# wenxuanliu/multimodal-vae

Measured on AMD Instinct MI355X. Metric: ELBO-steps/sec (whole node), MultiMNIST b=256 per GPU, higher is better.
Workload: dtype bf16; 1 GPU; multimnist_50x50_conv_mmvae_gru_text_3pass_elbo_step; batch_per_gpu=256, global_batch=256, n_latents=100, parallelism=dp1, hip_graph=False, optimizer=adam, mfma=bf16 in / fp32 acc; fp32 master weights, BN stats, PoE/KL/BCE/NLL, Adam

## Files before the change

### include/mmvae_hip.h

```cpp
#ifndef MMVAE_HIP_H
#define MMVAE_HIP_H
#include <stddef.h>
#include <stdint.h>

#ifdef __cplusplus
extern "C" {
#endif

#define MMVAE_OK 0
#define MMVAE_EINVAL (-1)
#define MMVAE_EHIP (-2)
#define MMVAE_ENOSPC (-3)
#define MMVAE_ESTATE (-4)
#define MMVAE_ETIMEOUT (-5)

int mmvae_init(int device);
const char* mmvae_last_error(void);
const char* mmvae_version(void);
int mmvae_set_stream_policy(int flat);

typedef struct mmvae_comm mmvae_comm_t;
int mmvae_comm_unique_id(void* out128);
int mmvae_comm_init(mmvae_comm_t** out, int rank, int world, const void* unique_id128);
int mmvae_allreduce_grads(mmvae_comm_t*, float* flat, size_t n, void* stream);
// ... 64 lines not shown
int mmvae_mm_image_decoder_fwd(mmvae_mm_t*, void* ws, size_t ws_bytes, const float* z, int training, float* recon,
                               void* stream);
int mmvae_mm_image_decoder_bwd(mmvae_mm_t*, void* ws, size_t ws_bytes, const float* d_recon, const float* recon,
                               float* dz, void* stream);
int mmvae_mm_text_encoder_fwd(mmvae_mm_t*, void* ws, size_t ws_bytes, const long long* text, float* out_mu_logvar,
                              void* stream);
int mmvae_mm_text_encoder_bwd(mmvae_mm_t*, void* ws, size_t ws_bytes, const long long* text, const float* d_out,
                              void* stream);
int mmvae_mm_text_decoder_fwd(mmvae_mm_t*, void* ws, size_t ws_bytes, const float* z, int training, const uint8_t* keep,
                              const long long* force_tokens, float* words, long long* tokens, void* stream);
int mmvae_mm_text_decoder_bwd(mmvae_mm_t*, void* ws, size_t ws_bytes, const float* z, const uint8_t* keep,
                              const long long* force_tokens, const float* words, const long long* tokens,
                              const float* d_words, float* dz, void* stream);
size_t mmvae_mm_iw_workspace_bytes(const mmvae_mm_t*);
int mmvae_mm_iw_score(mmvae_mm_t*, void* ws, size_t ws_bytes, const float* z, const float* image, int B, int K, float* loglik_x,
                      float* words, void* stream);
int mmvae_mm_bench_layer(mmvae_mm_t*, void* ws, size_t ws_bytes, const char* layer, int iters, void* stream);
double mmvae_mm_layer_flops(const mmvae_mm_t*, const char* layer);
double mmvae_mm_layer_algo_flops(const mmvae_mm_t*, const char* layer);
double mmvae_mm_layer_algo_bytes(const mmvae_mm_t*, const char* layer);
double mmvae_debug_flops(int reset);
int mmvae_debug_set(const char* key, int value);
long long mmvae_mm_debug_offset(mmvae_mm_t*, const char* name);

typedef struct MnistPlan mmvae_mnist_t;
mmvae_mnist_t* mmvae_mnist_create(int n_latents, int batch);
mmvae_mnist_t* mmvae_mnist_create_p(int n_latents, int batch, int precision);
int mmvae_mnist_precision(const mmvae_mnist_t*);
void mmvae_mnist_destroy(mmvae_mnist_t*);
long long mmvae_mnist_param_count(const mmvae_mnist_t*);
int mmvae_mnist_num_params(const mmvae_mnist_t*);
int mmvae_mnist_param_info(const mmvae_mnist_t*, int i, char* name128, int* ndim, int* shape4, long long* offset);
long long mmvae_mnist_bn_floats(const mmvae_mnist_t*);
int mmvae_mnist_num_bn(const mmvae_mnist_t*);
int mmvae_mnist_bn_info(const mmvae_mnist_t*, int i, char* prefix128, int* channels, long long* offset);
long long mmvae_mnist_packed_elems(const mmvae_mnist_t*);
long long mmvae_mnist_packed_vec_elems(const mmvae_mnist_t*);
long long mmvae_mnist_gpk_elems(const mmvae_mnist_t*);
long long mmvae_mnist_gpk_vec_elems(const mmvae_mnist_t*);
size_t mmvae_mnist_desc_bytes(const mmvae_mnist_t*, int which);
int mmvae_mnist_desc_copy(const mmvae_mnist_t*, int which, void* host_out);
size_t mmvae_mnist_workspace_bytes(const mmvae_mnist_t*);
size_t mmvae_mnist_module_workspace_bytes(const mmvae_mnist_t*);
int mmvae_mnist_bind(mmvae_mnist_t*, float* params, float* grads, float* bn_stats, long long* num_batches_tracked,
                     void* packed_bf16, float* packed_vec, float* gpk, float* gpk_vec, void* desc_dev, void* gdesc_dev);
int mmvae_mnist_pack_weights(mmvae_mnist_t*, void* stream);
// ... 446 lines not shown
```

### multimodal-vae_amd/csrc/capi.cpp

```cpp
#include "../../include/mmvae_hip.h"
#include "multimnist.h"
#include "mmtext.h"
#include "mnist.h"
#include "mnist_plan.h"
#include "mnist_strip.h"
#include "celeba.h"
#include "coco.h"
#include "plan_base.h"
#include "iw.h"
#include "nn_words.h"
#include "mmd.h"
#include "tsne.h"
#include "pixelcnn.h"
#include "causal_conv.h"
#include "head_nll.h"
#include "conv4s2.h"
#include "multimnist_gen.h"
#include "imgprep.h"
#include <cstring>
#include <exception>

const char* mmvae_error_string();

template <class F>
// ... 153 lines not shown
}
size_t mmvae_mm_iw_workspace_bytes(const mmvae_mm_t* p) { return mm_b(p)->ws_bytes_module; }
int mmvae_mm_iw_score(mmvae_mm_t* p, void* ws, size_t wsb, const float* z, const float* image, int B, int K, float* loglik_x,
                      float* words, void* stream) {
    return guarded([&] { return mm_iw_score(p, ws, wsb, z, image, B, K, loglik_x, words, S(stream)); });
}
int mmvae_mm_image_step(mmvae_mm_t* p, const mmvae_image_step_io* io, int training, int do_backward, void* stream) {
    return guarded([&]() -> int {
        MMVAE_REQUIRE(p && io, "mmvae_mm_image_step: null argument");
        return mm_image_step(p, *io, training, do_backward, S(stream));
    });
}
size_t mmvae_mm_image_step_workspace_bytes(const mmvae_mm_t* p) { return p ? mm_image_step_workspace_bytes(p) : 0; }
int mmvae_mm_iw_score_image(mmvae_mm_t* p, void* ws, size_t wsb, const float* z, const float* image, int B, int K, float* loglik_x, void* st) {
    return guarded([&] { return mm_iw_score_image(p, ws, wsb, z, image, B, K, loglik_x, S(st)); });
}
int mmvae_mm_bench_layer(mmvae_mm_t* p, void* ws, size_t wsb, const char* layer, int iters, void* stream) {
    return guarded([&] { return mm_bench_layer(p, ws, wsb, layer, iters, S(stream)); });
}
double mmvae_mm_layer_flops(const mmvae_mm_t* p, const char* layer) { return mm_layer_flops(p, layer); }
double mmvae_mm_layer_algo_flops(const mmvae_mm_t* p, const char* layer) { return mm_layer_algo_flops(p, layer); }
double mmvae_mm_layer_algo_bytes(const mmvae_mm_t* p, const char* layer) { return mm_layer_algo_bytes(p, layer); }
long long mmvae_mm_debug_offset(mmvae_mm_t* p, const char* name) { return mm_debug_offset(p, name); }

mmvae_mmtext_t* mmvae_mmtext_create(int n_latents, int n_hiddens, int batch) {
    try { return mmtext_create(n_latents, n_hiddens, batch); } catch (...) { mmvae_set_error("mmtext_create failed"); return nullptr; }
}
void mmvae_mmtext_destroy(mmvae_mmtext_t* p) { mmtext_destroy(p); }
int mmvae_mmtext_hidden(const mmvae_mmtext_t* p) { return mmtext_hidden(p); }
MMVAE_PLAN_API(mmtext, mmvae_mmtext_t, mmtext_b)
int mmvae_mmtext_step(mmvae_mmtext_t* p, const mmvae_mm_text_step_io* io, int training, int do_backward, void* stream) {
    return guarded([&]() -> int {
        MMVAE_REQUIRE(p && io, "mmvae_mmtext_step: null argument");
        return mmtext_step(p, *io, training, do_backward, S(stream));
    });
}
int mmvae_mmtext_encoder_fwd(mmvae_mmtext_t* p, void* ws, size_t wsb, const long long* text, float* out, void* stream) {
    return guarded([&] { return mmtext_encoder_fwd(p, ws, wsb, text, out, S(stream)); });
}
int mmvae_mmtext_encoder_bwd(mmvae_mmtext_t* p, void* ws, size_t wsb, const long long* text, const float* d_out, void* stream) {
    return guarded([&] { return mmtext_encoder_bwd(p, ws, wsb, text, d_out, S(stream)); });
}
int mmvae_mmtext_decoder_fwd(mmvae_mmtext_t* p, void* ws, size_t wsb, const float* z, int training, const uint8_t* keep,
                             const long long* force_tokens, float* words, long long* tokens, void* stream) {
    return guarded([&] { return mmtext_decoder_fwd(p, ws, wsb, z, training, keep, force_tokens, words, tokens, S(stream)); });
}
// ... 886 lines not shown
```

### multimodal-vae_amd/csrc/elementwise.h

```cpp
#pragma once
#include "common.h"

struct PackDesc {
    long long dst_off;
    long long src_off;
    int Npad, Kpad, N, K;
    int NL;
    int s_nhi, s_nlo;
    int TW, C;
    int s_ty, s_tx, s_c;
    int o_ty, o_tx, step_t;
    int is_f32;
    long long bias_off;
    int b_nhi, b_nlo;
    int first_block;
    int part;
    int frag;
};

int launch_pack(const PackDesc* table_dev, const PackDesc* table_host, int ndesc, const float* params,
                bf16* packed_bf, float* packed_f32, hipStream_t s);
int launch_pack_range(const PackDesc* table_dev, const PackDesc* table_host, int ndesc, int d0, int d1, const float* params,
                      bf16* packed_bf, float* packed_f32, hipStream_t s);
int launch_unpack_grads(const PackDesc* table_dev, const PackDesc* table_host, int ndesc, const float* gpk_mat,
                        const float* gpk_vec, float* grads_flat, hipStream_t s, int part = -1);

int launch_im2col_small(const float* src, int Nimg, int Cin, int H, int W, int KH, int KW, int stride, int pad,
                        int OH, int OW, bf16* dst, int ld, hipStream_t s);

struct BnFinalizeArgs {
    const float2* stats;
    int G, C;
    float count;
    const float* gamma; const float* beta;
    float* running_mean; float* running_var; long long* num_batches_tracked;
    int updates_per_group;
    unsigned skip_update_mask;
    float2* affine;
    float2* meanrstd;
    float eps, momentum;
    int training;
// ... 126 lines not shown
    const int* gmap; const float* gpk; const float* gpk_vec; float* g_out;
    int nr; long long roff[4], rlen[4]; int no_advance;
};
int launch_adam(const AdamArgs& a, hipStream_t s);
int launch_gather_rows(const void* src, const long long* idx, long long rows, long long row_bytes, void* dst, hipStream_t s);
int launch_gather_rows_u8_f32(const unsigned char* src, const long long* idx, long long rows, long long row_elems, float denom, float* dst, hipStream_t s);
struct StepLossArgs { const float* sums; float* out; float w_bce[3], w_nll[3], w_kl[3]; };
int launch_step_losses(const StepLossArgs& a, hipStream_t s);
int launch_unpack_map(const PackDesc* table_dev, const PackDesc* table_host, int nd, long long nparams, long long gmat_elems, int* map, hipStream_t s);
int launch_fill_zero(void* p, size_t bytes, hipStream_t s);
int launch_bce_fwd(const float* p, const float* t, long long n, float* out, hipStream_t s);
int launch_bce_bwd(const float* p, const float* t, long long n, float coef, const float* gscale, float* dp, hipStream_t s);
int launch_nll_fwd(const float* lp, const long long* tg, int rows, int classes, float* out, hipStream_t s);
int launch_nll_bwd(const long long* tg, int rows, int classes, float coef, const float* gscale, float* dlp, hipStream_t s);

struct StepBeginArgs {
    void* zero_ptr[4]; size_t zero_bytes[4];
    float* eps; long long n_eps;
    uint8_t* mask[3]; long long n_mask[3];
    float p;
    unsigned long long seed; const long long* step;
    const PackDesc* pack_table; int pack_nd; const float* pack_params; bf16* packed_bf; float* packed_f32; int pack_blocks;
    unsigned pack_parts;
};
int launch_step_begin(const StepBeginArgs& a, hipStream_t s);
int step_begin_with_pack(StepBeginArgs& a, const PackDesc* table_dev, const PackDesc* table_host, int nd, const float* params,
                         bf16* packed_bf, float* packed_f32);

int launch_embed_gather_stats(const float* table, int C, const long long* idx, int rows, int idx_rows, int rows_per_group,
                              bf16* x, int ld, float2* colstats, hipStream_t s);
int launch_embed_scatter_add(const bf16* d, int ld, int C, const long long* idx, int rows, float* g_table, hipStream_t s);
struct LogSoftmaxNllArgs {
    const float* logits; int rows, classes;
    float* words;
    const long long* target; int target_rows; int rows_per_group;
    float* nll_sum;
    bf16* dlogits; int ld_d;
    float* dlogits_f32;
    float coef[4];
};
int launch_logsoftmax_nll(const LogSoftmaxNllArgs& a, hipStream_t s);
int launch_cast_bf16(const float* x, long long n, bf16* out, hipStream_t s);
int launch_colsum_f32(const float* x, int rows, int cols, float* out, hipStream_t s);
int launch_colsum_bf16(const bf16* x, int ld, int rows, int cols, float* out, hipStream_t s);
int launch_u8_to_f32(const uint8_t* src, long long n, float denom, float* dst, hipStream_t s);
int launch_mse_fwd(const float* a, const float* b, long long n, float* out_sum, hipStream_t s);
int launch_mse_bwd(const float* a, const float* b, long long n, float coef, const float* gscale, float* d_a, hipStream_t s);
```

### multimodal-vae_amd/csrc/elementwise.hip

```cpp
#include "elementwise.h"
#include "bn_dev.h"
#include <math.h>

namespace {

constexpr int TPB = 256;

__device__ __forceinline__ float exp_unfused(float x) {
    const float c = 0x1.715476p+0f, cc = 0x1.4ae0bep-26f;
    float ph = x * c;
    asm volatile("" : "+v"(ph));
    float pl = fmaf(x, c, -ph);
    pl = fmaf(x, cc, pl);
    const float e = rintf(ph);
    float r = ldexpf(__builtin_amdgcn_exp2f((ph - e) + pl), (int)e);
    r = x < -0x1.9d1dap+6f ? 0.f : r;
    r = x > 0x1.62e43p+6f ? INFINITY : r;
    return r;
}
inline int nblocks(long long n, int per = TPB, int cap = 4096) {
    long long b = (n + per - 1) / per;
    if (b < 1) b = 1;
    if (b > cap) b = cap;
    return (int)b;
}

__device__ __forceinline__ int find_desc(const PackDesc* t, int nd, int block) {
    const int lane = threadIdx.x & 63;
    int found = 0;
    for (int base = 0; base < nd; base += 64) {
        const int i = base + lane;
        const bool le = i < nd && t[i].first_block <= block;
        const unsigned long long m = __ballot(le);
        found += __popcll(m);
        if (m != ~0ull) break;
    }
    return __builtin_amdgcn_readfirstlane(found > 0 ? found - 1 : 0);
}
__device__ __forceinline__ int fast_divmod_ew(int r, int d, float inv, int& rem) {
    int q = (int)((float)r * inv);
    rem = r - q * d;
    if (rem < 0) { --q; rem += d; }
    else if (rem >= d) { ++q; rem -= d; }
    return q;
}
__device__ __forceinline__ long long pack_src(const PackDesc& d, int n, int k) {
    int nhi = n / d.NL, nlo = n - nhi * d.NL;
    int tap = k / d.C, c = k - tap * d.C;
    int ty = tap / d.TW, tx = tap - ty * d.TW;
    return d.src_off + (long long)nhi * d.s_nhi + (long long)nlo * d.s_nlo +
           (long long)(d.o_ty + ty * d.step_t) * d.s_ty + (long long)(d.o_tx + tx * d.step_t) * d.s_tx + (long long)c * d.s_c;
}

__device__ __forceinline__ void pack_block(const PackDesc* __restrict__ table, int nd, const float* __restrict__ params,
                                           bf16* __restrict__ packed_bf, float* __restrict__ packed_f32, int block, unsigned parts = 0u) {
    const int di = find_desc(table, nd, block);
    const PackDesc d = table[di];
    if (parts != 0u && !((parts >> (d.part & 31)) & 1u)) return;
    const int v = (int)(block - d.first_block) * TPB + threadIdx.x;
    const int vpr = d.Kpad / 8;
    if (v >= d.Npad * vpr) return;
    int kv;
    const int n = fast_divmod_ew(v, vpr, 1.0f / (float)vpr, kv);
    const int k0 = kv * 8;
    float val[8];
#pragma unroll
    for (int j = 0; j < 8; ++j) val[j] = 0.f;
    if (n < d.N) {
        int nlo;
        const int nhi = fast_divmod_ew(n, d.NL, 1.0f / (float)d.NL, nlo);
        const long long rowbase = d.src_off + (long long)nhi * d.s_nhi + (long long)nlo * d.s_nlo;
        if (d.C % 8 == 0 && k0 + 8 <= d.K) {
            int c, tx;
            const int tap = fast_divmod_ew(k0, d.C, 1.0f / (float)d.C, c);
            const int ty = fast_divmod_ew(tap, d.TW, 1.0f / (float)d.TW, tx);
            const long long b = rowbase + (long long)(d.o_ty + ty * d.step_t) * d.s_ty + (long long)(d.o_tx + tx * d.step_t) * d.s_tx + (long long)c * d.s_c;
#pragma unroll
            for (int j = 0; j < 8; ++j) val[j] = params[b + (long long)j * d.s_c];
        } else {
#pragma unroll
            for (int j = 0; j < 8; ++j) {
                const int k = k0 + j;
                if (k < d.K) val[j] = params[pack_src(d, n, k)];
                else if (k == d.K && d.bias_off >= 0) val[j] = params[d.bias_off + (long long)nhi * d.b_nhi + (long long)nlo * d.b_nlo];
            }
        }
    }
    const long long e = d.frag ? ((long long)((n >> 4) * (d.Kpad >> 5) + (kv >> 2)) * 64 + (kv & 3) * 16 + (n & 15)) * 8 : (long long)n * d.Kpad + k0;
    if (d.is_f32) {
#pragma unroll
        for (int j = 0; j < 8; ++j) packed_f32[d.dst_off + e + j] = val[j];
    } else {
        bf16x8 o;
#pragma unroll
        for (int j = 0; j < 8; ++j) o[j] = (bf16)val[j];
        *reinterpret_cast<bf16x8*>(packed_bf + d.dst_off + e) = o;
    }
}

__global__ __launch_bounds__(TPB) void pack_kernel(const PackDesc* __restrict__ table, int nd, const float* __restrict__ params,
                                                   bf16* __restrict__ packed_bf, float* __restrict__ packed_f32, int block0) {
    pack_block(table, nd, params, packed_bf, packed_f32, block0 + blockIdx.x);
}

template <bool MAP>
__global__ __launch_bounds__(TPB) void unpack_kernel(const PackDesc* __restrict__ table, int nd, const float* __restrict__ gmat,
                                                     const float* __restrict__ gvec, float* __restrict__ grads, int* __restrict__ map,
                                                     int part) {
    const int di = find_desc(table, nd, blockIdx.x);
    const PackDesc d = table[di];
    if (part >= 0 && d.part != part) return;
    const int v = (int)(blockIdx.x - d.first_block) * TPB + threadIdx.x;
    const int vpr = d.Kpad / 8;
    if (v >= d.N * vpr) return;
    int kv, nlo;
    const int n = fast_divmod_ew(v, vpr, 1.0f / (float)vpr, kv);
    const int k0 = kv * 8;
    if (k0 > d.K) return;
    const int nhi = fast_divmod_ew(n, d.NL, 1.0f / (float)d.NL, nlo);
    const long long sidx = d.dst_off + (long long)n * d.Kpad + k0;
    float val[8] = {0.f, 0.f, 0.f, 0.f, 0.f, 0.f, 0.f, 0.f};
    if (!MAP) {
        const float* src = (d.is_f32 ? gvec : gmat) + sidx;
        const f32x4 lo = *reinterpret_cast<const f32x4*>(src), hi = *reinterpret_cast<const f32x4*>(src + 4);
#pragma unroll
// ... 307 lines not shown
    for (long long q = (long long)blockIdx.x * TPB + threadIdx.x; q * 4 < n; q += (long long)gridDim.x * TPB) {
        uint32_t r[4];
        Philox::gen(seed ^ (st * 0x9E3779B97F4A7C15ull), (uint64_t)q, stream_id, r);
        float u0 = u01(r[0]), u1 = u01(r[1]), u2 = u01(r[2]), u3 = u01(r[3]);
        float m0 = sqrtf(-2.0f * logf(u0)), m1 = sqrtf(-2.0f * logf(u2));
        float v[4] = {m0 * cosf(6.28318530718f * u1), m0 * sinf(6.28318530718f * u1),
                      m1 * cosf(6.28318530718f * u3), m1 * sinf(6.28318530718f * u3)};
        for (int j = 0; j < 4; ++j)
            if (q * 4 + j < n) out[q * 4 + j] = v[j];
    }
}
__global__ __launch_bounds__(TPB) void keep_mask_kernel(uint8_t* out, long long n, float p, unsigned long long seed, const long long* step, unsigned stream_id) {
    const unsigned long long st = step ? (unsigned long long)*step : 0ull;
    for (long long q = (long long)blockIdx.x * TPB + threadIdx.x; q * 4 < n; q += (long long)gridDim.x * TPB) {
        uint32_t r[4];
        Philox::gen(seed ^ (st * 0x9E3779B97F4A7C15ull), (uint64_t)q, stream_id, r);
        for (int j = 0; j < 4; ++j)
            if (q * 4 + j < n) out[q * 4 + j] = u01(r[j]) >= p ? 1 : 0;
    }
}

__global__ __launch_bounds__(TPB) void step_begin_kernel(const StepBeginArgs a) {
    if ((int)blockIdx.x < a.pack_blocks) {
        pack_block(a.pack_table, a.pack_nd, a.pack_params, a.packed_bf, a.packed_f32, blockIdx.x, a.pack_parts);
        return;
    }
    const long long gtid = (long long)(blockIdx.x - a.pack_blocks) * TPB + threadIdx.x, gstride = (long long)(gridDim.x - a.pack_blocks) * TPB;
#pragma unroll
    for (int r = 0; r < 4; ++r) {
        if (!a.zero_ptr[r]) continue;
        u32x4* p = reinterpret_cast<u32x4*>(a.zero_ptr[r]);
        const long long n16 = (long long)(a.zero_bytes[r] / 16);
        for (long long i = gtid; i < n16; i += gstride) p[i] = u32x4{0u, 0u, 0u, 0u};
    }
    const unsigned long long st = a.step ? (unsigned long long)*a.step : 0ull;
    const unsigned long long key = a.seed ^ (st * 0x9E3779B97F4A7C15ull);
    if (a.eps) {
        for (long long q = gtid; q * 4 < a.n_eps; q += gstride) {
            uint32_t r[4];
            Philox::gen(key, (uint64_t)q, 1, r);
            float u0 = u01(r[0]), u1 = u01(r[1]), u2 = u01(r[2]), u3 = u01(r[3]);
            float m0 = sqrtf(-2.0f * logf(u0)), m1 = sqrtf(-2.0f * logf(u2));
            float v[4] = {m0 * cosf(6.28318530718f * u1), m0 * sinf(6.28318530718f * u1),
                          m1 * cosf(6.28318530718f * u3), m1 * sinf(6.28318530718f * u3)};
            for (int j = 0; j < 4; ++j)
                if (q * 4 + j < a.n_eps) a.eps[q * 4 + j] = v[j];
        }
// ... 489 lines not shown
}

}

int launch_mse_fwd(const float* a, const float* b, long long n, float* out, hipStream_t s) {
    hipLaunchKernelGGL(mse_fwd_kernel, dim3(nblocks(n, TPB * 4, 256)), dim3(TPB), 0, s, a, b, n, out);
    return mmvae_check_launch("mse_fwd");
}
int launch_mse_bwd(const float* a, const float* b, long long n, float coef, const float* gs, float* da, hipStream_t s) {
    hipLaunchKernelGGL(mse_bwd_kernel, dim3((unsigned)((n + TPB - 1) / TPB)), dim3(TPB), 0, s, a, b, n, coef, gs, da);
    return mmvae_check_launch("mse_bwd");
}
int launch_u8_to_f32(const uint8_t* src, long long n, float denom, float* dst, hipStream_t s) {
    MMVAE_REQUIRE(src && dst && n >= 0, "u8_to_f32: null argument");
    if (n == 0) return MMVAE_OK;
    hipLaunchKernelGGL(u8_to_f32_kernel, dim3((unsigned)((n + 16 * TPB - 1) / (16 * TPB))), dim3(TPB), 0, s, src, n, denom, dst);
    return mmvae_check_launch("u8_to_f32");
}
int launch_pack(const PackDesc* table_dev, const PackDesc* table_host, int nd, const float* params, bf16* packed_bf,
                float* packed_f32, hipStream_t s) {
    MMVAE_REQUIRE(nd > 0, "pack: empty table");
    for (int i = 0; i < nd; ++i)
        MMVAE_REQUIRE((long long)table_host[i].Npad * (table_host[i].Kpad / 8) < (1 << 23), "pack: matrix %d too large for 32-bit index math", i);
    hipLaunchKernelGGL(pack_kernel, dim3(table_blocks(table_host, nd)), dim3(TPB), 0, s, table_dev, nd, params, packed_bf, packed_f32, 0);
    return mmvae_check_launch("pack");
}
int launch_pack_range(const PackDesc* table_dev, const PackDesc* table_host, int nd, int d0, int d1, const float* params, bf16* packed_bf,
                      float* packed_f32, hipStream_t s) {
    MMVAE_REQUIRE(0 <= d0 && d0 <= d1 && d1 <= nd, "pack: descriptor range [%d, %d) of %d", d0, d1, nd);
    if (d0 == d1) return MMVAE_OK;
    const int b0 = (int)table_host[d0].first_block, b1 = d1 < nd ? (int)table_host[d1].first_block : table_blocks(table_host, nd);
    hipLaunchKernelGGL(pack_kernel, dim3(b1 - b0), dim3(TPB), 0, s, table_dev, nd, params, packed_bf, packed_f32, b0);
    return mmvae_check_launch("pack");
}
int launch_unpack_grads(const PackDesc* table_dev, const PackDesc* table_host, int nd, const float* gmat, const float* gvec,
                        float* grads, hipStream_t s, int part) {
    MMVAE_REQUIRE(nd > 0, "unpack: empty table");
    for (int i = 0; i < nd; ++i)
        MMVAE_REQUIRE((long long)table_host[i].Npad * (table_host[i].Kpad / 8) < (1 << 23), "unpack: matrix %d too large for 32-bit index math", i);
    hipLaunchKernelGGL(unpack_kernel<false>, dim3(table_blocks(table_host, nd)), dim3(TPB), 0, s, table_dev, nd, gmat, gvec, grads, (int*)nullptr, part);
    return mmvae_check_launch("unpack_grads");
}
int launch_unpack_map(const PackDesc* table_dev, const PackDesc* table_host, int nd, long long nparams, long long gmat_elems, int* map, hipStream_t s) {
    MMVAE_REQUIRE(nd > 0 && map, "unpack_map: empty table");
    MMVAE_REQUIRE(gmat_elems < (1ll << 31) - 2, "unpack_map: packed gradient buffer too large for 32-bit indices");
    if (hipMemsetAsync(map, 0xFF, (size_t)nparams * sizeof(int), s) != hipSuccess) { mmvae_set_error("hipMemsetAsync failed"); return MMVAE_EHIP; }
    hipLaunchKernelGGL(unpack_kernel<true>, dim3(table_blocks(table_host, nd)), dim3(TPB), 0, s, table_dev, nd, (const float*)nullptr,
                       (const float*)nullptr, (float*)nullptr, map, -1);
    return mmvae_check_launch("unpack_map");
}
int launch_im2col_small(const float* src, int Nimg, int Cin, int H, int W, int KH, int KW, int stride, int pad, int OH, int OW,
                        bf16* dst, int ld, hipStream_t s) {
    MMVAE_REQUIRE(ld % 8 == 0 && ld >= KH * KW * Cin && ld / 8 <= TPB, "im2col: ld=%d", ld);
    MMVAE_REQUIRE((long long)Nimg * OH * OW < (1 << 23) && (long long)Cin * H * W < (1ll << 31), "im2col: too many rows");
    const int rpb = TPB / (ld / 8);
// ... 215 lines not shown
    return MMVAE_OK;
}

int launch_bce_fwd(const float* p, const float* t, long long n, float* out, hipStream_t s) {
    hipLaunchKernelGGL(bce_fwd_kernel, dim3(nblocks(n, TPB * 4, 1024)), dim3(TPB), 0, s, p, t, n, out);
    return mmvae_check_launch("bce_fwd");
}
int launch_bce_bwd(const float* p, const float* t, long long n, float coef, const float* gs, float* dp, hipStream_t s) {
    hipLaunchKernelGGL(bce_bwd_kernel, dim3((unsigned)((n + TPB - 1) / TPB)), dim3(TPB), 0, s, p, t, n, coef, gs, dp);
    return mmvae_check_launch("bce_bwd");
}
int launch_nll_fwd(const float* lp, const long long* tg, int rows, int classes, float* out, hipStream_t s) {
    hipLaunchKernelGGL(nll_fwd_kernel, dim3(nblocks(rows, TPB, 64)), dim3(TPB), 0, s, lp, tg, rows, classes, out);
    return mmvae_check_launch("nll_fwd");
}
int launch_nll_bwd(const long long* tg, int rows, int classes, float coef, const float* gs, float* dlp, hipStream_t s) {
    hipLaunchKernelGGL(nll_bwd_kernel, dim3(ceil_div(rows * classes, TPB)), dim3(TPB), 0, s, tg, rows, classes, coef, gs, dlp);
    return mmvae_check_launch("nll_bwd");
}

int launch_step_begin(const StepBeginArgs& a, hipStream_t s) {
    for (int r = 0; r < 4; ++r)
        MMVAE_REQUIRE(a.zero_ptr[r] == nullptr || (a.zero_bytes[r] % 16 == 0 && ((uintptr_t)a.zero_ptr[r] & 15) == 0), "step_begin: zero range %d is not 16-byte aligned", r);
    MMVAE_LAUNCH(step_begin_kernel, dim3(mmvae_knob("begin_blocks", 2048) + (a.pack_blocks > 0 ? a.pack_blocks : 0)), dim3(TPB), 0, s, a);
    return mmvae_check_launch("step_begin");
}
int step_begin_with_pack(StepBeginArgs& a, const PackDesc* table_dev, const PackDesc* table_host, int nd, const float* params,
                         bf16* packed_bf, float* packed_f32) {
    MMVAE_REQUIRE(nd > 0, "pack: empty table");
    for (int i = 0; i < nd; ++i)
        MMVAE_REQUIRE((long long)table_host[i].Npad * (table_host[i].Kpad / 8) < (1 << 23), "pack: matrix %d too large for 32-bit index math", i);
    a.pack_table = table_dev; a.pack_nd = nd; a.pack_params = params; a.packed_bf = packed_bf; a.packed_f32 = packed_f32;
    a.pack_blocks = table_blocks(table_host, nd);
    return MMVAE_OK;
}

int launch_embed_gather_stats(const float* table, int C, const long long* idx, int rows, int idx_rows, int rows_per_group,
                              bf16* x, int ld, float2* colstats, hipStream_t s) {
    MMVAE_REQUIRE(C >= 1 && ld >= C && ld % 8 == 0, "embed_gather: C=%d ld=%d", C, ld);
    MMVAE_REQUIRE(rows >= 1 && idx_rows >= 1 && rows_per_group >= 1 && table && idx && x, "embed_gather: rows=%d idx_rows=%d rows_per_group=%d or a null argument",
                  rows, idx_rows, rows_per_group);
    hipLaunchKernelGGL(embed_gather_stats_kernel, dim3(ceil_div(rows, 64)), dim3(TPB), 0, s, table, C, idx, rows, idx_rows, rows_per_group, x, ld, colstats);
    return mmvae_check_launch("embed_gather_stats");
}
int launch_embed_scatter_add(const bf16* d, int ld, int C, const long long* idx, int rows, float* g_table, hipStream_t s) {
    MMVAE_REQUIRE(rows >= 1 && C >= 1 && ld >= C && (long long)rows * C <= 0x3FFFFFFF && d && idx && g_table, "embed_scatter: rows=%d C=%d ld=%d or a null argument",
                  rows, C, ld);
    hipLaunchKernelGGL(embed_scatter_add_kernel, dim3(ceil_div(rows * C, TPB)), dim3(TPB), 0, s, d, ld, C, idx, rows, g_table);
    return mmvae_check_launch("embed_scatter_add");
}
int launch_logsoftmax_nll(const LogSoftmaxNllArgs& a, hipStream_t s) {
    MMVAE_REQUIRE(a.rows >= 1 && a.classes >= 1 && a.rows_per_group >= 1 && a.logits && a.words, "logsoftmax_nll: rows=%d classes=%d rows_per_group=%d or a null argument",
                  a.rows, a.classes, a.rows_per_group);
    MMVAE_REQUIRE(ceil_div(a.rows, a.rows_per_group) <= 4, "logsoftmax_nll: %d rows are more than 4 groups of %d", a.rows, a.rows_per_group);
    MMVAE_REQUIRE(!a.target || a.target_rows >= 1, "logsoftmax_nll: target_rows=%d", a.target_rows);
    MMVAE_REQUIRE(!a.dlogits || a.ld_d >= a.classes, "logsoftmax_nll: ld_d=%d < classes=%d", a.ld_d, a.classes);
// ... 23 lines not shown
```

### multimodal-vae_amd/csrc/multimnist.h

```cpp
#pragma once
#include "layers.h"
#include "text.h"
#include "../../include/mmvae_hip.h"

struct PlanBase;

struct MMPlan;
int mm_early_ranges(const MMPlan* P, long long* ranges, int cap);
MMPlan* mm_create(int D, int B);
void mm_destroy(MMPlan*);
PlanBase* mm_base(MMPlan*);
int mm_step_fwd_bwd(MMPlan*, const mmvae_mm_step_io&, int training, int do_backward, hipStream_t);
int mm_image_encoder_fwd(MMPlan*, void* ws, size_t wsb, const float* image, const uint8_t* m1, const uint8_t* m2,
                         int training, float* out, hipStream_t);
int mm_image_encoder_bwd(MMPlan*, void* ws, size_t wsb, const float* d_out, const uint8_t* m1, const uint8_t* m2, hipStream_t);
int mm_image_decoder_fwd(MMPlan*, void* ws, size_t wsb, const float* z, int training, float* recon, hipStream_t);
int mm_image_decoder_bwd(MMPlan*, void* ws, size_t wsb, const float* d_recon, const float* recon, float* dz, hipStream_t);
int mm_text_encoder_fwd(MMPlan*, void* ws, size_t wsb, const long long* text, float* out, hipStream_t);
int mm_text_encoder_bwd(MMPlan*, void* ws, size_t wsb, const long long* text, const float* d_out, hipStream_t);
int mm_text_decoder_fwd(MMPlan*, void* ws, size_t wsb, const float* z, int training, const uint8_t* keep,
                        const long long* force_tokens, float* words, long long* tokens, hipStream_t);
int mm_text_decoder_bwd(MMPlan*, void* ws, size_t wsb, const float* z, const uint8_t* keep, const long long* force_tokens,
                        const float* words, const long long* tokens, const float* d_words, float* dz, hipStream_t);
int mm_iw_score(MMPlan*, void* ws, size_t wsb, const float* z, const float* image, int B, int K, float* loglik_x, float* words,
                hipStream_t);
int mm_image_step(MMPlan*, const mmvae_image_step_io&, int training, int do_backward, hipStream_t);
size_t mm_image_step_workspace_bytes(const MMPlan*);
int mm_iw_score_image(MMPlan*, void* ws, size_t wsb, const float* z, const float* image, int B, int K, float* loglik_x, hipStream_t);
int mm_wait_early_grads(MMPlan*, hipStream_t s);
int mm_bench_layer(MMPlan*, void* ws, size_t wsb, const char* layer, int iters, hipStream_t);
double mm_layer_flops(const MMPlan*, const char* layer);
double mm_layer_algo_flops(const MMPlan*, const char* layer);
double mm_layer_algo_bytes(const MMPlan*, const char* layer);
long long mm_debug_offset(MMPlan*, const char* name);
```

### multimodal-vae_amd/csrc/multimnist.hip

```cpp
#include "multimnist.h"
#include <memory>
#include "mlp_tail.h"
#include "plan_base.h"
#include "thin.h"
#include "text_plan.h"
#include <cstring>

namespace {
constexpr int IMG = 50, NPIX = 2500;
}

struct MMPlan : PlanBase {
    int ldz, kx, kz;
    int lde;
    ConvL conv[4], convT[4];
    LinL fc[3], up;
    BnL bn[6];
    int H = TXT_H;
    const char *te_name = "text_encoder", *td_name = "text_decoder";
    TextGruIdx te_f, te_r, td0, td1;
    const float* step_image = nullptr;
    hipEvent_t ev_dz = nullptr;
    hipEvent_t ev_txtgrads = nullptr;
    int te_h2p, te_h2pT, g_te_h2p, td_z2h, td_z2hT, g_td_z2h, td_h2o, td_h2oT, g_td_h2o;
// ... 705 lines not shown
    const uint8_t *m1 = io.enc_mask1, *m2 = io.enc_mask2, *gk = io.gru_keep;
    const bool serial0 = mmvae_serial();
    const bool staged = mmvae_knob("mm_stage_begin", 1) != 0 && !serial0;
    StepBeginArgs sb{}, sb2{};
    sb.zero_ptr[0] = w.zero_begin; sb.zero_bytes[0] = w.zero_bytes;
    StepBeginArgs& sz = staged ? sb2 : sb;
    if (do_backward) {
        sz.zero_ptr[1] = P.buf.gpk; sz.zero_bytes[1] = (size_t)P.gk.mat_elems * sizeof(float);
        sz.zero_ptr[2] = P.buf.grads; sz.zero_bytes[2] = (size_t)(P.nparams / 4) * 16;
        const int skipz = mmvae_knob("dbg_begin_skip_zero", 0);
        if (skipz & 1) sz.zero_ptr[1] = nullptr;
        if (skipz & 2) sz.zero_ptr[2] = nullptr;
    }
    sb.p = DROP_P; sb.seed = io.seed; sb.step = io.step_counter;
    if (training && !eps) { sb.eps = w.eps; sb.n_eps = (long long)B3 * D; eps = w.eps; }
    if (training && io.enc_dropout && !m1) { sb.mask[0] = w.m1; sb.n_mask[0] = (long long)2 * B * 400; m1 = w.m1; }
    if (training && io.enc_dropout && !m2) { sb.mask[1] = w.m2; sb.n_mask[1] = (long long)2 * B * 200; m2 = w.m2; }
    if (training && io.gru_dropout && !gk) { sb.mask[2] = w.gkeep; sb.n_mask[2] = (long long)4 * B3 * P.H; gk = w.gkeep; }
    const int skipb = mmvae_knob("dbg_begin_skip", 0);
    if (skipb & 2) { sb.eps = nullptr; sb.mask[0] = sb.mask[1] = sb.mask[2] = nullptr; }
    if (skipb & 4) sb.zero_ptr[0] = nullptr;
    const bool pack_now = io.pack_first && !(skipb & 1);
    if (pack_now) {
        MMVAE_TRY(step_begin_with_pack(sb, P.buf.desc_dev, P.pk.d.data(), (int)P.pk.d.size(), P.buf.params, P.buf.packed, P.buf.packed_vec));
        if (staged) sb.pack_parts = 1u << 0;
    }
    MMVAE_TRY(ensure_streams(P));
    P.in_step = true;
    {
        hipStreamCaptureStatus cs = hipStreamCaptureStatusNone;
        P.capturing = hipStreamIsCapturing(s, &cs) == hipSuccess && cs == hipStreamCaptureStatusActive;
    }
    arm_fork(P);
    MMVAE_TRY(launch_step_begin(sb, s));
    MMVAE_TRY(commit_fork(P, s));
    if (do_backward && P.nparams % 4 != 0)
        MMVAE_TRY(launch_fill_zero(P.buf.grads + (P.nparams / 4) * 4, (size_t)(P.nparams % 4) * sizeof(float), s));
    const int enc_drop = training && io.enc_dropout;
    const int sk[3] = {io.pass_skip[0] != 0, io.pass_skip[1] != 0, io.pass_skip[2] != 0};
    P.dec_skip_mask = (unsigned)(sk[0] | (sk[1] << 1) | (sk[2] << 2));
    const int enc_updates = 2 - sk[0] - sk[1];
    const bool serial = mmvae_serial();
    hipStream_t T = serial ? s : P.st_text;
    if (T != s) MMVAE_TRY(fork_to(P, T));
    if (staged && pack_now) {
        StepBeginArgs st1{};
        MMVAE_TRY(step_begin_with_pack(st1, P.buf.desc_dev, P.pk.d.data(), (int)P.pk.d.size(), P.buf.params, P.buf.packed, P.buf.packed_vec));
        st1.pack_parts = 1u << 1;
        MMVAE_TRY(launch_step_begin(st1, T));
    }
    {
        TextEncArgs a = te_args(P, io.text, w.txtout, do_backward);
        MMVAE_TRY(launch_text_encoder_fwd(a, T));
    }
    if (staged && (pack_now || sb2.zero_ptr[1] || sb2.zero_ptr[2])) {
        if (pack_now) {
            MMVAE_TRY(step_begin_with_pack(sb2, P.buf.desc_dev, P.pk.d.data(), (int)P.pk.d.size(), P.buf.params, P.buf.packed, P.buf.packed_vec));
            sb2.pack_parts = 1u << 2;
        }
        MMVAE_TRY(launch_step_begin(sb2, T));
    }
    P.step_image = io.image;
    const bool fuse = mmvae_knob("mm_fuse_bn", 1) != 0 && mmvae_knob("convres", 1) != 0 && B % 8 == 0;
    MMVAE_TRY(enc_fwd(P, io.image, 2, m1, m2, enc_drop, training, enc_updates, w.encout, s, fuse));
    MMVAE_TRY(edge(P, T, s));
    Latent3Args la{};
    la.B = B; la.D = D; la.img_out = w.encout; la.txt_out = w.txtout; la.eps = eps;
    la.mu = io.mu ? io.mu : w.mu; la.logvar = io.logvar ? io.logvar : w.logvar;
    la.z_f32 = w.z_f32; la.z_bf = w.z_bf; la.ldz = P.ldz; la.kl_sum = w.sums + 8; la.training = training;
    arm_fork(P);
    MMVAE_TRY(launch_latent3_fwd(la, s));
    MMVAE_TRY(commit_fork(P, s));
    if (T != s) MMVAE_TRY(fork_to(P, T));
    TextDecArgs td = td_args(P, w.z_f32, 3, do_backward);
    td.keep = (training && io.gru_dropout) ? gk : nullptr; td.keep_scale = 1.f / (1.f - DROP_P);
    td.force_tokens = io.force_tokens;
    if (io.recon_text) td.words = io.recon_text;
    if (io.tokens) td.tokens_out = io.tokens;
    td.target = io.text; td.nll_sum = w.sums + 4; td.dwords = do_backward ? w.dwords : nullptr;
    for (int k = 0; k < 3; ++k) td.nll_coef[k] = sk[k] ? 0.f : io.lambda_yx[k] / (float)(B * TXT_T);
    if (const int half = mmvae_knob("dbg_text_rows_div", 0)) td.R = max(16, td.R / half);
    MMVAE_TRY(launch_text_decoder_fwd(td, T));
// ... 548 lines not shown
}
double mm_layer_algo_bytes(const MMPlan* Pc, const char* layer) {
    const MMPlan& P = *Pc;
    const std::string name = layer;
    const int B = P.B;
    auto conv = [&](const ConvL& L, int images, bool wgrad) {
        const ConvGeom& g = L.g;
        const double act = (double)images * ((double)g.IH * g.IW * g.Cin + (double)g.OH * g.OW * g.Cout) * 2.0;
        return act + (double)g.Cin * g.Cout * g.KH * g.KW * (wgrad ? 4.0 : 2.0);
    };
    for (int l = 0; l < 4; ++l) {
        const std::string e = "enc_conv" + std::to_string(l + 1), d = "dec_convT" + std::to_string(l + 1);
        if (name == e || name == e + "_dgrad") return conv(P.conv[l], B, false);
        if (name == e + "_wgrad") return conv(P.conv[l], B, true);
        if (name == d) return conv(P.convT[l], 3 * B, false);
        if (name == d + "_dgrad") return conv(P.convT[l], 2 * B, false);
        if (name == d + "_wgrad") return conv(P.convT[l], 2 * B, true);
    }
    if (name == "enc_conv1_mfma") return (double)B * (2500 * 4.0 + 2 * 625 * 32 * 2.0) + 32 * 16 * 2.0;
    if (name == "enc_conv1_wgrad_mfma") return (double)B * (2500 * 4.0 + 625 * 32 * 2.0) + 32 * 16 * 4.0;
    if (name == "dec_last_fused" || name == "dec_last_fused_reduce") return 2.0 * B * (2 * 625 * 32 * 2.0 + 2500 * 4.0) + 32 * 16 * 4.0;
    return 0.0;
}
long long mm_debug_offset(MMPlan* P, const char* name) {
    Workspace ws((void*)0x1000, (size_t)1 << 40);
    const bool one_pass = std::strncmp(name, "image_step:", 11) == 0;
    if (one_pass) name += 11;
    P->carve_passes = one_pass ? 1 : 3;
    carve(*P, ws);
    P->carve_passes = 3;
    MMPlan::W& w = P->w;
    std::map<std::string, const void*> m = {
        {"patches1", w.patches1}, {"r1", w.r1}, {"r2", w.r2}, {"r3", w.r3}, {"r4", w.r4}, {"y1", w.y1}, {"y2", w.y2},
        {"encout", w.encout}, {"txtout", w.txtout}, {"z_bf", w.z_bf}, {"z_f32", w.z_f32}, {"u", w.u}, {"q1", w.q1}, {"q2", w.q2},
        {"q3", w.q3}, {"logits", w.logits}, {"dlogit", w.dlogit}, {"d3", w.d3}, {"d2", w.d2}, {"d1", w.d1}, {"du", w.du},
        {"dz_img", w.dz_img}, {"dz_txt", w.dz_txt}, {"d_encout", w.d_encout}, {"d_txtout", w.d_txtout}, {"dy2", w.dy2},
        {"dy1", w.dy1}, {"db4", w.db4}, {"dr4", w.dr4}, {"d3e", w.d3e}, {"d2e", w.d2e}, {"d1e", w.d1e},
        {"aff_d0", w.aff_d[0]}, {"aff_d1", w.aff_d[1]}, {"aff_d2", w.aff_d[2]}, {"st_d0", w.st_d[0]}, {"patches4", w.patches4},
        {"tmp_f32", w.tmp_f32}, {"aff_e0", w.aff_e[0]}, {"aff_e1", w.aff_e[1]}, {"aff_e2", w.aff_e[2]},
        {"eps", w.eps}, {"m1", w.m1}, {"m2", w.m2}, {"gkeep", w.gkeep},
        {"st_e0", w.st_e[0]}, {"st_e1", w.st_e[1]}, {"st_e2", w.st_e[2]}, {"st_d1", w.st_d[1]}, {"st_d2", w.st_d[2]},
        {"red_e0", w.red_e[0]}, {"red_e1", w.red_e[1]}, {"red_e2", w.red_e[2]},
        {"red_d0", w.red_d[0]}, {"red_d1", w.red_d[1]}, {"red_d2", w.red_d[2]},
        {"a1", w.a1}, {"a2", w.a2}, {"a3", w.a3}, {"aq1", w.aq1}, {"aq2", w.aq2}, {"aq3", w.aq3},
        {"a4", w.a4}, {"au", w.au}, {"ay1", w.ay1}, {"ay2", w.ay2}, {"slab", w.slab},
        {"mr_e0", w.mr_e[0]}, {"mr_e1", w.mr_e[1]}, {"mr_e2", w.mr_e[2]}, {"mr_d0", w.mr_d[0]}, {"mr_d1", w.mr_d[1]}, {"mr_d2", w.mr_d[2]},
// ... 7 lines not shown
```

Measured before the change: 1790 ELBO-steps/s.

## Reorder weight-pack gathers along the smallest source stride and size staged pack grids

Adds a run-based path to the parameter pack kernel. For each descriptor it picks the loop axis (tap, output row, channel group) with the smallest source stride and assigns wave lanes along it, so the gather reads from the fp32 master params become coalesced; padding zeros are written in a separate loop. Staged step_begin launches now cover only the blocks of the selected part, using a range remap table, and the zero-fill grid is sized to the actual work instead of a fixed block count. This adds decode arithmetic per task and a 48-entry range table in the kernel arguments.

```diff
diff --git a/include/mmvae_hip.h b/include/mmvae_hip.h
--- a/include/mmvae_hip.h
+++ b/include/mmvae_hip.h
@@ -110,6 +110,7 @@
 double mmvae_debug_flops(int reset);
 int mmvae_debug_set(const char* key, int value);
 long long mmvae_mm_debug_offset(mmvae_mm_t*, const char* name);
+int mmvae_mm_debug_pack_stage(mmvae_mm_t*, int stage, int* blocks, void* stream);
 
 typedef struct MnistPlan mmvae_mnist_t;
 mmvae_mnist_t* mmvae_mnist_create(int n_latents, int batch);
diff --git a/multimodal-vae_amd/csrc/capi.cpp b/multimodal-vae_amd/csrc/capi.cpp
--- a/multimodal-vae_amd/csrc/capi.cpp
+++ b/multimodal-vae_amd/csrc/capi.cpp
@@ -199,6 +199,10 @@
 double mmvae_mm_layer_algo_flops(const mmvae_mm_t* p, const char* layer) { return mm_layer_algo_flops(p, layer); }
 double mmvae_mm_layer_algo_bytes(const mmvae_mm_t* p, const char* layer) { return mm_layer_algo_bytes(p, layer); }
 long long mmvae_mm_debug_offset(mmvae_mm_t* p, const char* name) { return mm_debug_offset(p, name); }
+int mmvae_mm_debug_pack_stage(mmvae_mm_t* p, int stage, int* blocks, void* stream) {
+    MMVAE_REQUIRE(p && stage >= -1 && stage <= 2, "debug_pack_stage: null plan or stage %d", stage);
+    return mm_debug_pack_stage(p, stage, blocks, (hipStream_t)stream);
+}
 
 mmvae_mmtext_t* mmvae_mmtext_create(int n_latents, int n_hiddens, int batch) {
     try { return mmtext_create(n_latents, n_hiddens, batch); } catch (...) { mmvae_set_error("mmtext_create failed"); return nullptr; }
diff --git a/multimodal-vae_amd/csrc/elementwise.h b/multimodal-vae_amd/csrc/elementwise.h
--- a/multimodal-vae_amd/csrc/elementwise.h
+++ b/multimodal-vae_amd/csrc/elementwise.h
@@ -1,22 +1,6 @@
 #pragma once
 #include "common.h"
-
-struct PackDesc {
-    long long dst_off;
-    long long src_off;
-    int Npad, Kpad, N, K;
-    int NL;
-    int s_nhi, s_nlo;
-    int TW, C;
-    int s_ty, s_tx, s_c;
-    int o_ty, o_tx, step_t;
-    int is_f32;
-    long long bias_off;
-    int b_nhi, b_nlo;
-    int first_block;
-    int part;
-    int frag;
-};
+#include "pack_geo.h"
 
 int launch_pack(const PackDesc* table_dev, const PackDesc* table_host, int ndesc, const float* params,
                 bf16* packed_bf, float* packed_f32, hipStream_t s);
@@ -189,10 +173,14 @@
     unsigned long long seed; const long long* step;
     const PackDesc* pack_table; int pack_nd; const float* pack_params; bf16* packed_bf; float* packed_f32; int pack_blocks;
     unsigned pack_parts;
-};
+    int pack_runs;
+    int pack_nr;
+    struct PackRange { int blk0, tb0; } pack_rng[48];
+};
+constexpr int STEP_BEGIN_MAX_RANGES = 48;
 int launch_step_begin(const StepBeginArgs& a, hipStream_t s);
 int step_begin_with_pack(StepBeginArgs& a, const PackDesc* table_dev, const PackDesc* table_host, int nd, const float* params,
-                         bf16* packed_bf, float* packed_f32);
+                         bf16* packed_bf, float* packed_f32, unsigned parts = 0u);
 
 int launch_embed_gather_stats(const float* table, int C, const long long* idx, int rows, int idx_rows, int rows_per_group,
                               bf16* x, int ld, float2* colstats, hipStream_t s);
diff --git a/multimodal-vae_amd/csrc/elementwise.hip b/multimodal-vae_amd/csrc/elementwise.hip
--- a/multimodal-vae_amd/csrc/elementwise.hip
+++ b/multimodal-vae_amd/csrc/elementwise.hip
@@ -44,19 +44,48 @@
     else if (rem >= d) { ++q; rem -= d; }
     return q;
 }
-__device__ __forceinline__ long long pack_src(const PackDesc& d, int n, int k) {
-    int nhi = n / d.NL, nlo = n - nhi * d.NL;
-    int tap = k / d.C, c = k - tap * d.C;
-    int ty = tap / d.TW, tx = tap - ty * d.TW;
-    return d.src_off + (long long)nhi * d.s_nhi + (long long)nlo * d.s_nlo +
-           (long long)(d.o_ty + ty * d.step_t) * d.s_ty + (long long)(d.o_tx + tx * d.step_t) * d.s_tx + (long long)c * d.s_c;
+__device__ __forceinline__ void pack_store(const PackDesc& d, bf16* __restrict__ packed_bf, float* __restrict__ packed_f32, long long e,
+                                           const float (&val)[8]) {
+    if (d.is_f32) {
+#pragma unroll
+        for (int j = 0; j < 8; ++j) packed_f32[d.dst_off + e + j] = val[j];
+    } else {
+        bf16x8 o;
+#pragma unroll
+        for (int j = 0; j < 8; ++j) o[j] = (bf16)val[j];
+        *reinterpret_cast<bf16x8*>(packed_bf + d.dst_off + e) = o;
+    }
+}
+__device__ __forceinline__ void pack_block_runs(const PackDesc& d, const PackRuns& g, const float* __restrict__ params,
+                                                bf16* __restrict__ packed_bf, float* __restrict__ packed_f32, int block) {
+    const int nb = pg_blocks(d), lb = block - d.first_block;
+    const int lane = threadIdx.x & (PG_WAVE - 1);
+    for (int task = pg_first_task(lb, threadIdx.x >> 6); task < g.tasks; task += pg_task_step(nb)) {
+        int n, tap, co;
+        if (!pg_runs_decode(g, task, lane, n, tap, co)) continue;
+        const long long b = pack_src(d, n, tap * d.C + co * 8);
+        float val[8];
+#pragma unroll
+        for (int j = 0; j < 8; ++j) val[j] = params[b + (long long)j * d.s_c];
+        pack_store(d, packed_bf, packed_f32, pack_dst(d, n, tap * g.CO + co), val);
+    }
+    const float zero[8] = {0.f, 0.f, 0.f, 0.f, 0.f, 0.f, 0.f, 0.f};
+    for (int i = lb * TPB + threadIdx.x; i < g.zeros; i += nb * TPB) {
+        int n, kv;
+        pg_zero_decode(d, g, i, n, kv);
+        pack_store(d, packed_bf, packed_f32, pack_dst(d, n, kv), zero);
+    }
 }
 
 __device__ __forceinline__ void pack_block(const PackDesc* __restrict__ table, int nd, const float* __restrict__ params,
-                                           bf16* __restrict__ packed_bf, float* __restrict__ packed_f32, int block, unsigned parts = 0u) {
+                                           bf16* __restrict__ packed_bf, float* __restrict__ packed_f32, int block, unsigned parts, int runs) {
     const int di = find_desc(table, nd, block);
     const PackDesc d = table[di];
     if (parts != 0u && !((parts >> (d.part & 31)) & 1u)) return;
+    if (runs) {
+        const PackRuns g = pg_runs(d);
+        if (g.ok) { pack_block_runs(d, g, params, packed_bf, packed_f32, block); return; }
+    }
     const int v = (int)(block - d.first_block) * TPB + threadIdx.x;
     const int vpr = d.Kpad / 8;
     if (v >= d.Npad * vpr) return;
@@ -99,8 +128,8 @@
 }
 
 __global__ __launch_bounds__(TPB) void pack_kernel(const PackDesc* __restrict__ table, int nd, const float* __restrict__ params,
-                                                   bf16* __restrict__ packed_bf, float* __restrict__ packed_f32, int block0) {
-    pack_block(table, nd, params, packed_bf, packed_f32, block0 + blockIdx.x);
+                                                   bf16* __restrict__ packed_bf, float* __restrict__ packed_f32, int block0, int runs) {
+    pack_block(table, nd, params, packed_bf, packed_f32, block0 + blockIdx.x, 0u, runs);
 }
 
 template <bool MAP>
@@ -454,7 +483,13 @@
 
 __global__ __launch_bounds__(TPB) void step_begin_kernel(const StepBeginArgs a) {
     if ((int)blockIdx.x < a.pack_blocks) {
-        pack_block(a.pack_table, a.pack_nd, a.pack_params, a.packed_bf, a.packed_f32, blockIdx.x, a.pack_parts);
+        int tb = blockIdx.x;
+        if (a.pack_nr > 0) {
+            int r = 0;
+            while (r + 1 < a.pack_nr && tb >= a.pack_rng[r + 1].blk0) ++r;
+            tb = tb - a.pack_rng[r].blk0 + a.pack_rng[r].tb0;
+        }
+        pack_block(a.pack_table, a.pack_nd, a.pack_params, a.packed_bf, a.packed_f32, tb, a.pack_parts, a.pack_runs);
         return;
     }
     const long long gtid = (long long)(blockIdx.x - a.pack_blocks) * TPB + threadIdx.x, gstride = (long long)(gridDim.x - a.pack_blocks) * TPB;
@@ -990,7 +1025,8 @@
     MMVAE_REQUIRE(nd > 0, "pack: empty table");
     for (int i = 0; i < nd; ++i)
         MMVAE_REQUIRE((long long)table_host[i].Npad * (table_host[i].Kpad / 8) < (1 << 23), "pack: matrix %d too large for 32-bit index math", i);
-    hipLaunchKernelGGL(pack_kernel, dim3(table_blocks(table_host, nd)), dim3(TPB), 0, s, table_dev, nd, params, packed_bf, packed_f32, 0);
+    hipLaunchKernelGGL(pack_kernel, dim3(table_blocks(table_host, nd)), dim3(TPB), 0, s, table_dev, nd, params, packed_bf, packed_f32, 0,
+                       mmvae_knob("pack_runs", 1));
     return mmvae_check_launch("pack");
 }
 int launch_pack_range(const PackDesc* table_dev, const PackDesc* table_host, int nd, int d0, int d1, const float* params, bf16* packed_bf,
@@ -998,7 +1034,7 @@
     MMVAE_REQUIRE(0 <= d0 && d0 <= d1 && d1 <= nd, "pack: descriptor range [%d, %d) of %d", d0, d1, nd);
     if (d0 == d1) return MMVAE_OK;
     const int b0 = (int)table_host[d0].first_block, b1 = d1 < nd ? (int)table_host[d1].first_block : table_blocks(table_host, nd);
-    hipLaunchKernelGGL(pack_kernel, dim3(b1 - b0), dim3(TPB), 0, s, table_dev, nd, params, packed_bf, packed_f32, b0);
+    hipLaunchKernelGGL(pack_kernel, dim3(b1 - b0), dim3(TPB), 0, s, table_dev, nd, params, packed_bf, packed_f32, b0, mmvae_knob("pack_runs", 1));
     return mmvae_check_launch("pack");
 }
 int launch_unpack_grads(const PackDesc* table_dev, const PackDesc* table_host, int nd, const float* gmat, const float* gvec,
@@ -1260,16 +1296,41 @@
 int launch_step_begin(const StepBeginArgs& a, hipStream_t s) {
     for (int r = 0; r < 4; ++r)
         MMVAE_REQUIRE(a.zero_ptr[r] == nullptr || (a.zero_bytes[r] % 16 == 0 && ((uintptr_t)a.zero_ptr[r] & 15) == 0), "step_begin: zero range %d is not 16-byte aligned", r);
-    MMVAE_LAUNCH(step_begin_kernel, dim3(mmvae_knob("begin_blocks", 2048) + (a.pack_blocks > 0 ? a.pack_blocks : 0)), dim3(TPB), 0, s, a);
+    long long items = 0;
+    for (int r = 0; r < 4; ++r)
+        if (a.zero_ptr[r]) items += (long long)(a.zero_bytes[r] / 16);
+    if (a.eps) items += (a.n_eps + 3) / 4;
+    for (int m = 0; m < 3; ++m)
+        if (a.mask[m]) items += (a.n_mask[m] + 3) / 4;
+    const int cap = mmvae_knob("begin_blocks", 2048);
+    const int begin = mmvae_knob("pack_stage_grid", 1) == 0 ? cap : items > 0 ? nblocks(items, TPB * 4, cap > 0 ? cap : 1) : 0;
+    const int pack = a.pack_blocks > 0 ? a.pack_blocks : 0;
+    if (begin + pack == 0) return MMVAE_OK;
+    MMVAE_LAUNCH(step_begin_kernel, dim3(begin + pack), dim3(TPB), 0, s, a);
     return mmvae_check_launch("step_begin");
 }
 int step_begin_with_pack(StepBeginArgs& a, const PackDesc* table_dev, const PackDesc* table_host, int nd, const float* params,
-                         bf16* packed_bf, float* packed_f32) {
+                         bf16* packed_bf, float* packed_f32, unsigned parts) {
     MMVAE_REQUIRE(nd > 0, "pack: empty table");
     for (int i = 0; i < nd; ++i)
         MMVAE_REQUIRE((long long)table_host[i].Npad * (table_host[i].Kpad / 8) < (1 << 23), "pack: matrix %d too large for 32-bit index math", i);
     a.pack_table = table_dev; a.pack_nd = nd; a.pack_params = params; a.packed_bf = packed_bf; a.packed_f32 = packed_f32;
+    a.pack_runs = mmvae_knob("pack_runs", 1);
     a.pack_blocks = table_blocks(table_host, nd);
+    a.pack_parts = parts; a.pack_nr = 0;
+    if (parts == 0u || mmvae_knob("pack_stage_grid", 1) == 0) return MMVAE_OK;
+    int nr = 0, blocks = 0;
+    bool fits = true;
+    for (int i = 0; i < nd && fits; ++i) {
+        if (!((parts >> (table_host[i].part & 31)) & 1u)) continue;
+        const bool cont = i > 0 && ((parts >> (table_host[i - 1].part & 31)) & 1u);
+        if (!cont) {
+            if (nr == STEP_BEGIN_MAX_RANGES) { fits = false; break; }
+            a.pack_rng[nr].blk0 = blocks; a.pack_rng[nr].tb0 = table_host[i].first_block; ++nr;
+        }
+        blocks += pg_blocks(table_host[i]);
+    }
+    if (fits) { a.pack_nr = nr; a.pack_blocks = blocks; a.pack_parts = nr > 0 ? 0u : parts; }
     return MMVAE_OK;
 }
 
diff --git a/multimodal-vae_amd/csrc/multimnist.h b/multimodal-vae_amd/csrc/multimnist.h
--- a/multimodal-vae_amd/csrc/multimnist.h
+++ b/multimodal-vae_amd/csrc/multimnist.h
@@ -33,3 +33,4 @@
 double mm_layer_algo_flops(const MMPlan*, const char* layer);
 double mm_layer_algo_bytes(const MMPlan*, const char* layer);
 long long mm_debug_offset(MMPlan*, const char* name);
+int mm_debug_pack_stage(MMPlan*, int stage, int* blocks, hipStream_t);
diff --git a/multimodal-vae_amd/csrc/multimnist.hip b/multimodal-vae_amd/csrc/multimnist.hip
--- a/multimodal-vae_amd/csrc/multimnist.hip
+++ b/multimodal-vae_amd/csrc/multimnist.hip
@@ -751,8 +751,8 @@
     if (skipb & 4) sb.zero_ptr[0] = nullptr;
     const bool pack_now = io.pack_first && !(skipb & 1);
     if (pack_now) {
-        MMVAE_TRY(step_begin_with_pack(sb, P.buf.desc_dev, P.pk.d.data(), (int)P.pk.d.size(), P.buf.params, P.buf.packed, P.buf.packed_vec));
-        if (staged) sb.pack_parts = 1u << 0;
+        MMVAE_TRY(step_begin_with_pack(sb, P.buf.desc_dev, P.pk.d.data(), (int)P.pk.d.size(), P.buf.params, P.buf.packed, P.buf.packed_vec,
+                                       staged ? 1u << 0 : 0u));
     }
     MMVAE_TRY(ensure_streams(P));
     P.in_step = true;
@@ -774,8 +774,7 @@
     if (T != s) MMVAE_TRY(fork_to(P, T));
     if (staged && pack_now) {
         StepBeginArgs st1{};
-        MMVAE_TRY(step_begin_with_pack(st1, P.buf.desc_dev, P.pk.d.data(), (int)P.pk.d.size(), P.buf.params, P.buf.packed, P.buf.packed_vec));
-        st1.pack_parts = 1u << 1;
+        MMVAE_TRY(step_begin_with_pack(st1, P.buf.desc_dev, P.pk.d.data(), (int)P.pk.d.size(), P.buf.params, P.buf.packed, P.buf.packed_vec, 1u << 1));
         MMVAE_TRY(launch_step_begin(st1, T));
     }
     {
@@ -783,10 +782,8 @@
         MMVAE_TRY(launch_text_encoder_fwd(a, T));
     }
     if (staged && (pack_now || sb2.zero_ptr[1] || sb2.zero_ptr[2])) {
-        if (pack_now) {
-            MMVAE_TRY(step_begin_with_pack(sb2, P.buf.desc_dev, P.pk.d.data(), (int)P.pk.d.size(), P.buf.params, P.buf.packed, P.buf.packed_vec));
-            sb2.pack_parts = 1u << 2;
-        }
+        if (pack_now)
+            MMVAE_TRY(step_begin_with_pack(sb2, P.buf.desc_dev, P.pk.d.data(), (int)P.pk.d.size(), P.buf.params, P.buf.packed, P.buf.packed_vec, 1u << 2));
         MMVAE_TRY(launch_step_begin(sb2, T));
     }
     P.step_image = io.image;
@@ -1381,6 +1378,14 @@
     if (name == "dec_last_fused" || name == "dec_last_fused_reduce") return 2.0 * B * (2 * 625 * 32 * 2.0 + 2500 * 4.0) + 32 * 16 * 4.0;
     return 0.0;
 }
+int mm_debug_pack_stage(MMPlan* Pp, int stage, int* blocks, hipStream_t s) {
+    MMPlan& P = *Pp;
+    StepBeginArgs sb{};
+    MMVAE_TRY(step_begin_with_pack(sb, P.buf.desc_dev, P.pk.d.data(), (int)P.pk.d.size(), P.buf.params, P.buf.packed, P.buf.packed_vec,
+                                   stage < 0 ? 0u : 1u << stage));
+    if (blocks) *blocks = sb.pack_blocks;
+    return launch_step_begin(sb, s);
+}
 long long mm_debug_offset(MMPlan* P, const char* name) {
     Workspace ws((void*)0x1000, (size_t)1 << 40);
     const bool one_pass = std::strncmp(name, "image_step:", 11) == 0;
diff --git a/multimodal-vae_amd/csrc/pack_geo.h b/multimodal-vae_amd/csrc/pack_geo.h
--- /dev/null
+++ b/multimodal-vae_amd/csrc/pack_geo.h
@@ -0,0 +1,117 @@
+#pragma once
+
+#if defined(__HIPCC__)
+#define PG_HD __host__ __device__ inline
+#else
+#define PG_HD inline
+#endif
+
+struct PackDesc {
+    long long dst_off;
+    long long src_off;
+    int Npad, Kpad, N, K;
+    int NL;
+    int s_nhi, s_nlo;
+    int TW, C;
+    int s_ty, s_tx, s_c;
+    int o_ty, o_tx, step_t;
+    int is_f32;
+    long long bias_off;
+    int b_nhi, b_nlo;
+    int first_block;
+    int part;
+    int frag;
+};
+
+constexpr int PG_TPB = 256, PG_WAVE = 64, PG_WAVES = PG_TPB / PG_WAVE;
+
+PG_HD int pg_divmod(int r, int d, int& rem) {
+    int q = (int)((float)r * (1.0f / (float)d));
+    rem = r - q * d;
+    if (rem < 0) { --q; rem += d; }
+    else if (rem >= d) { ++q; rem -= d; }
+    return q;
+}
+
+PG_HD long long pg_vectors(const PackDesc& d) { return (long long)d.Npad * (d.Kpad / 8); }
+PG_HD int pg_blocks(const PackDesc& d) { return (int)((pg_vectors(d) + PG_TPB - 1) / PG_TPB); }
+
+PG_HD long long pack_src(const PackDesc& d, int n, int k) {
+    int nhi = n / d.NL, nlo = n - nhi * d.NL;
+    int tap = k / d.C, c = k - tap * d.C;
+    int ty = tap / d.TW, tx = tap - ty * d.TW;
+    return d.src_off + (long long)nhi * d.s_nhi + (long long)nlo * d.s_nlo +
+           (long long)(d.o_ty + ty * d.step_t) * d.s_ty + (long long)(d.o_tx + tx * d.step_t) * d.s_tx + (long long)c * d.s_c;
+}
+PG_HD long long pack_bias_src(const PackDesc& d, int n) {
+    int nhi = n / d.NL, nlo = n - nhi * d.NL;
+    return d.bias_off + (long long)nhi * d.b_nhi + (long long)nlo * d.b_nlo;
+}
+PG_HD long long pack_dst(const PackDesc& d, int n, int kv) {
+    return d.frag ? ((long long)((n >> 4) * (d.Kpad >> 5) + (kv >> 2)) * 64 + (kv & 3) * 16 + (n & 15)) * 8 : (long long)n * d.Kpad + kv * 8;
+}
+
+enum { PG_TAP = 0, PG_N = 1, PG_CO = 2 };
+struct PackRuns {
+    int ok;
+    int T, CO;
+    int ax[3], ext[3];
+    int E, G, segs;
+    int units, tasks;
+    int vpr, padv;
+    int zrows, zeros;
+};
+
+PG_HD long long pg_stride_mag(long long s) { return s < 0 ? -s : (s == 0 ? (1ll << 40) : s); }
+
+PG_HD PackRuns pg_runs(const PackDesc& d) {
+    PackRuns r{};
+    if (d.s_c == 1 || d.C < 8 || d.C % 8 != 0 || d.bias_off >= 0 || d.is_f32 || d.K <= 0 || d.K % d.C != 0 || d.TW < 1 || d.N < 1 || d.N > d.Npad) return r;
+    r.T = d.K / d.C; r.CO = d.C / 8;
+    if (r.T % d.TW != 0 || r.T > PG_WAVE) return r;
+    const long long huge = 1ll << 40;
+    long long st[3];
+    st[PG_TAP] = r.T > 1 ? pg_stride_mag((long long)(d.TW > 1 ? d.s_tx : d.s_ty) * d.step_t) : huge;
+    st[PG_N] = d.N > 1 ? pg_stride_mag(d.NL > 1 ? d.s_nlo : d.s_nhi) : huge;
+    st[PG_CO] = r.CO > 1 ? pg_stride_mag(8ll * d.s_c) : huge;
+    const int full[3] = {r.T, d.N, r.CO};
+    int a0 = 0, a1 = 1, a2 = 2;
+    if (st[a1] < st[a0]) { int t = a0; a0 = a1; a1 = t; }
+    if (st[a2] < st[a1]) { int t = a1; a1 = a2; a2 = t; }
+    if (st[a1] < st[a0]) { int t = a0; a0 = a1; a1 = t; }
+    r.ax[0] = a0; r.ax[1] = a1; r.ax[2] = a2;
+    for (int i = 0; i < 3; ++i) r.ext[i] = full[r.ax[i]];
+    if (r.ext[0] <= PG_WAVE) { r.E = r.ext[0]; r.G = PG_WAVE / r.E; r.segs = 1; }
+    else { r.segs = (r.ext[0] + PG_WAVE - 1) / PG_WAVE; r.E = (r.ext[0] + r.segs - 1) / r.segs; r.G = 1; }
+    const long long units = (long long)r.segs * r.ext[1] * r.ext[2];
+    if (units >= (1 << 23)) return r;
+    r.units = (int)units; r.tasks = (r.units + r.G - 1) / r.G;
+    r.vpr = d.Kpad / 8; r.padv = r.vpr - r.T * r.CO;
+    r.zrows = (d.Npad - d.N) * r.vpr; r.zeros = r.zrows + d.N * r.padv;
+    r.ok = 1;
+    return r;
+}
+
+PG_HD bool pg_runs_decode(const PackRuns& r, int task, int lane, int& n, int& tap, int& co) {
+    int e;
+    const int g = pg_divmod(lane, r.E, e);
+    int u = task * r.G + g;
+    if (g >= r.G || u >= r.units) return false;
+    int idx[3], seg = 0;
+    if (r.segs > 1) u = pg_divmod(u, r.segs, seg);
+    idx[0] = seg * r.E + e;
+    if (idx[0] >= r.ext[0]) return false;
+    idx[2] = pg_divmod(u, r.ext[1], idx[1]);
+    int out[3];
+    for (int i = 0; i < 3; ++i) out[r.ax[i]] = idx[i];
+    tap = out[PG_TAP]; n = out[PG_N]; co = out[PG_CO];
+    return true;
+}
+PG_HD void pg_zero_decode(const PackDesc& d, const PackRuns& r, int i, int& n, int& kv) {
+    if (i < r.zrows) { n = d.N + pg_divmod(i, r.vpr, kv); return; }
+    int p;
+    n = pg_divmod(i - r.zrows, r.padv, p);
+    kv = r.T * r.CO + p;
+}
+PG_HD int pg_first_task(int lb, int wave) { return lb * PG_WAVES + wave; }
+PG_HD int pg_task_step(int nb) { return nb * PG_WAVES; }
```

Measured after the change: 1821 ELBO-steps/s (median of 6 runs). +1.7%, better.
